# IDEA-CCNL/Fengshenbang-LM

Hardware: AMD Instinct MI355X
Metric: tokens/sec Ziya-LLaMA-13B ZeRO-3 (higher is better)
Workload: dtype bf16; 1 GPU; model=Ziya-LLaMA-13B, global_batch=16, micro_batch=16, seq_len=2048, parallelism=zero3_dp1, activation_checkpointing=True, ckpt_skip_interval=4

## Files before the change

### fengshen_amd/ops/csrc/bindings.cpp

```cpp
#include <torch/extension.h>

#include <hip/hip_runtime.h>
#include <c10/hip/HIPStream.h>

#include <string>
#include <vector>

enum FsDtype { FS_F32 = 0, FS_BF16 = 1, FS_F16 = 2 };

static int fs_dtype(const at::Tensor& t) {
  switch (t.scalar_type()) {
    case at::kFloat: return FS_F32;
    case at::kBFloat16: return FS_BF16;
    case at::kHalf: return FS_F16;
    default: TORCH_CHECK(false, "unsupported dtype ", t.scalar_type());
  }
}

static hipStream_t cur_stream() {
  return c10::hip::getCurrentHIPStream().stream();
}

extern "C" {
void fs_rms_norm_fwd(const void*, const void*, void*, float*, int, int, float,
                     int, hipStream_t);
void fs_rms_norm_bwd(const void*, const void*, const void*, const float*,
                     void*, float*, int, int, int, hipStream_t);
void fs_layer_norm_fwd(const void*, const void*, const void*, void*, float*,
                       float*, int, int, float, int, hipStream_t);
void fs_layer_norm_bwd(const void*, const void*, const void*, const float*,
                       const float*, void*, float*, float*, int, int, int,
                       hipStream_t);
void fs_scaled_softmax_fwd(const void*, const unsigned char*, void*, float,
                           int, int, int, int, int, int, int, int,
                           hipStream_t);
void fs_scaled_softmax_bwd(const void*, const void*, void*, float, int, int,
                           int, hipStream_t);
void fs_rope(const void*, void*, const float*, const float*, long, int, int,
             int, int, int, hipStream_t);
void fs_swiglu_fwd(const void*, void*, long, int, int, hipStream_t);
void fs_swiglu_bwd(const void*, const void*, void*, long, int, int,
                   hipStream_t);
void fs_bias_gelu(const void*, const void*, const void*, void*, long, int, int,
                  int, hipStream_t);
void fs_fused_adamw(float*, const void*, float*, float*, void*, long, float,
                    float, float, float, float, int, int, int, hipStream_t);
void fs_flash_attn_fwd(const void*, const void*, const void*, void*, float*,
                       const int*, int, int, int, int, int, int, float,
                       float, unsigned long long, hipStream_t);
void fs_flash_attn_bwd(const void*, const void*, const void*, const void*,
                       const void*, const float*, void*, void*, void*, float*,
                       const int*, int, int, int, int, int, int, float,
                       float, unsigned long long, hipStream_t);
void fs_bf16_gemv(const void*, const void*, void*, int, int, int,
                  hipStream_t);
void fs_add_rms_norm(const void*, const void*, const void*, void*, void*,
                     int, int, float, hipStream_t);
void fs_decode_attn(const void*, void*, void*, const float*, const float*,
                    const void*, void*, int, int, int, int, int, float, int,
                    hipStream_t);
void fs_w8_gemv(const void*, const float*, const void*, void*, int, int, int,
                hipStream_t);
void fs_vocab_ce_fwd(const void*, const long*, float*, float*, float*,
                     long, int, int, int, hipStream_t);
void fs_vocab_ce_bwd(const void*, const long*, const float*, const float*,
                     const float*, void*, long, int, int, int, hipStream_t);
void fs_flash_attn_fwd_v3(const void*, const void*, const void*, void*,
                          float*, const int*, int, int, int, int, int, float,
                          float, unsigned long long, hipStream_t);
void fs_flash_attn_bwd_v3(const void*, const void*, const void*, const void*,
                          const void*, const float*, void*, void*, void*,
                          float*, const int*, int, int, int, int, int, float,
                          float, unsigned long long, hipStream_t);
void fs_flash_attn_fwd_v3_strided(const void*, const void*, const void*,
                                  void*, float*, const int*, const long*,
                                  const long*, int, int, int, int, int, float,
                                  float, unsigned long long, hipStream_t);
void fs_flash_attn_bwd_v3_strided(const void*, const void*, const void*,
                                  const void*, const void*, const float*,
                                  void*, void*, void*, float*, const int*,
                                  const long*, const long*, const long*,
                                  const long*, int, int, int, int, int, float,
                                  float, unsigned long long, hipStream_t);
void fs_flash_attn_fwd_v3_kstart(const void*, const void*, const void*, void*,
                                 float*, const int*, const long*, const long*,
                                 int, int, int, int, float, hipStream_t);
void fs_flash_attn_bwd_v3_kstart(const void*, const void*, const void*,
                                 const void*, const void*, const float*,
                                 void*, void*, void*, float*, const int*,
// ... 497 lines not shown
  }
  if (kstart.has_value()) {
    fs_flash_attn_fwd_v3_kstart(q.data_ptr(), k.data_ptr(), v.data_ptr(),
                                o.data_ptr(), lse.data_ptr<float>(),
                                kstart->data_ptr<int>(), qs, os, b, h, s, d,
                                (float)scale, cur_stream());
    return lse;
  }
  fs_flash_attn_fwd_v3_strided(q.data_ptr(), k.data_ptr(), v.data_ptr(),
                               o.data_ptr(), lse.data_ptr<float>(), klp, qs,
                               os, b, h, s, d, causal ? 1 : 0, (float)scale,
                               0.f, 0ull, cur_stream());
  return lse;
}

static void flash_attn_bwd_v3_strided(
    at::Tensor q, at::Tensor k, at::Tensor v, at::Tensor o, at::Tensor dout,
    at::Tensor lse, at::Tensor dq, at::Tensor dk, at::Tensor dv, double scale,
    bool causal, c10::optional<at::Tensor> klens,
    c10::optional<at::Tensor> kstart, c10::optional<at::Tensor> qend,
    bool check_values) {
  TORCH_CHECK(q.dim() == 4, "q must be [b, h, s, d]");
  const int b = q.size(0), h = q.size(1), s = q.size(2), d = q.size(3);
  TORCH_CHECK((d == 128 || d == 96 || d == 64) && s % 64 == 0 && s >= 64,
              "flash v3: d in {64, 96, 128}, s a multiple of 64");
  const int h_kv = checked_kv_heads(k, h, causal, 0.0, klens.has_value());
  check_strided_view(q, "q", b, h, s, d);
  check_strided_view(k, "k", b, h_kv, s, d);
  check_strided_view(v, "v", b, h_kv, s, d);
  check_strided_view(o, "o", b, h, s, d);
  check_strided_view(dout, "dout", b, h, s, d);
  check_strided_view(dq, "dq", b, h, s, d);
  check_strided_view(dk, "dk", b, h_kv, s, d);
  check_strided_view(dv, "dv", b, h_kv, s, d);
  if (h_kv == h) {
    check_same_strides(q, k, "q and k");
    check_same_strides(dq, dk, "dq and dk");
  }
  check_same_strides(k, v, "k and v");
  check_same_strides(dk, dv, "dk and dv");
  TORCH_CHECK(lse.is_cuda() && lse.scalar_type() == at::kFloat &&
              lse.is_contiguous() && lse.numel() == (int64_t)b * h * s,
              "lse must be contiguous fp32 [b, h, s]");
  if (kstart.has_value())
    check_kstart(*kstart, qend, true, q, causal, 0.0, klens.has_value(),
                 check_values);
  else
    TORCH_CHECK(!qend.has_value(), "flash v3: qend without kstart");
  const int* klp = checked_klens(klens, causal, b);
  long qs[3], os[3], dos[3], gs[3];
  strides3(q, qs);
  strides3(o, os);
  strides3(dout, dos);
  strides3(dq, gs);
  auto delta = at::empty({b, h, s}, q.options().dtype(at::kFloat));
  if (h_kv != h) {
    long kvs[3], gkvs[3];
    strides3(k, kvs);
    strides3(dk, gkvs);
    const bool ks = kstart.has_value();
    fs_flash_attn_bwd_v3_gqa(
        q.data_ptr(), k.data_ptr(), v.data_ptr(), o.data_ptr(),
        dout.data_ptr(), lse.data_ptr<float>(), dq.data_ptr(), dk.data_ptr(),
        dv.data_ptr(), delta.data_ptr<float>(),
        ks ? kstart->data_ptr<int>() : nullptr,
        ks ? qend->data_ptr<int>() : nullptr, qs, kvs, os, dos, gs, gkvs, b,
        h, h_kv, s, d, (float)scale, cur_stream());
    return;
  }
  if (kstart.has_value()) {
    fs_flash_attn_bwd_v3_kstart(
        q.data_ptr(), k.data_ptr(), v.data_ptr(), o.data_ptr(),
        dout.data_ptr(), lse.data_ptr<float>(), dq.data_ptr(), dk.data_ptr(),
        dv.data_ptr(), delta.data_ptr<float>(), kstart->data_ptr<int>(),
        qend->data_ptr<int>(), qs, os, dos, gs, b, h, s, d, (float)scale,
        cur_stream());
    return;
  }
  fs_flash_attn_bwd_v3_strided(
      q.data_ptr(), k.data_ptr(), v.data_ptr(), o.data_ptr(), dout.data_ptr(),
      lse.data_ptr<float>(), dq.data_ptr(), dk.data_ptr(), dv.data_ptr(),
      delta.data_ptr<float>(), klp, qs, os, dos, gs, b, h, s, d,
      causal ? 1 : 0, (float)scale, 0.f, 0ull, cur_stream());
}

static void rope_inplace(at::Tensor q, at::Tensor k, at::Tensor cos,
                         at::Tensor sin, int64_t offset, bool bwd) {
  TORCH_CHECK(q.dim() == 4, "q must be [b, np, s, hn]");
  const int b = q.size(0), np = q.size(1), s = q.size(2), hn = q.size(3);
  TORCH_CHECK((hn / 2) % 8 == 0 && hn % 2 == 0,
              "head_dim/2 must be divisible by 8");
  check_strided_view(q, "q", b, np, s, hn);
  check_strided_view(k, "k", b, np, s, hn);
  check_same_strides(q, k, "q and k");
  TORCH_CHECK(cos.is_cuda() && sin.is_cuda() &&
              cos.scalar_type() == at::kFloat &&
              sin.scalar_type() == at::kFloat && cos.is_contiguous() &&
              sin.is_contiguous() && cos.dim() == 2 && cos.size(1) == hn &&
              sin.sizes() == cos.sizes(),
              "cos/sin must be contiguous fp32 [S, hn]");
  TORCH_CHECK(offset >= 0 && offset + s <= cos.size(0),
              "rope table too short for offset + s");
  fs_rope_inplace(q.data_ptr(), k.data_ptr(), cos.data_ptr<float>(),
                  sin.data_ptr<float>(), b, np, s, hn, q.stride(0),
                  q.stride(1), q.stride(2), (int)offset, bwd ? 1 : 0,
                  fs_dtype(q), cur_stream());
}

static void rope_inplace_one(at::Tensor x, at::Tensor cos, at::Tensor sin,
                             int64_t offset, bool bwd) {
  TORCH_CHECK(x.dim() == 4, "x must be [b, n, s, hn]");
  const int b = x.size(0), np = x.size(1), s = x.size(2), hn = x.size(3);
  TORCH_CHECK((hn / 2) % 8 == 0 && hn % 2 == 0,
              "head_dim/2 must be divisible by 8");
  check_strided_view(x, "x", b, np, s, hn);
  TORCH_CHECK(cos.is_cuda() && sin.is_cuda() &&
              cos.scalar_type() == at::kFloat &&
              sin.scalar_type() == at::kFloat && cos.is_contiguous() &&
              sin.is_contiguous() && cos.dim() == 2 && cos.size(1) == hn &&
              sin.sizes() == cos.sizes(),
              "cos/sin must be contiguous fp32 [S, hn]");
  TORCH_CHECK(offset >= 0 && offset + s <= cos.size(0),
              "rope table too short for offset + s");
  fs_rope_inplace(x.data_ptr(), nullptr, cos.data_ptr<float>(),
                  sin.data_ptr<float>(), b, np, s, hn, x.stride(0),
                  x.stride(1), x.stride(2), (int)offset, bwd ? 1 : 0,
                  fs_dtype(x), cur_stream());
}

static at::Tensor w8_gemv(at::Tensor q8, at::Tensor scale, at::Tensor x) {
  TORCH_CHECK(q8.scalar_type() == at::kChar && x.scalar_type() == at::kBFloat16);
  TORCH_CHECK(q8.is_contiguous() && x.is_contiguous());
  const int out = q8.size(0), in = q8.size(1);
  TORCH_CHECK(in % 16 == 0, "in_features must be divisible by 16");
  const int b = x.numel() / in;
  auto y = at::empty({b, out}, x.options());
  fs_w8_gemv(q8.data_ptr(), scale.data_ptr<float>(), x.data_ptr(),
             y.data_ptr(), b, in, out, cur_stream());
  return y;
}

static at::Tensor bf16_gemv(at::Tensor w, at::Tensor x) {
  TORCH_CHECK(w.scalar_type() == at::kBFloat16 &&
              x.scalar_type() == at::kBFloat16);
  TORCH_CHECK(w.is_contiguous() && x.is_contiguous());
  const int out = w.size(0), in = w.size(1);
  TORCH_CHECK(in % 16 == 0, "in_features must be divisible by 16");
  const int b = x.numel() / in;
  TORCH_CHECK(b >= 1 && b <= 8, "bf16_gemv: batch must be 1..8");
  auto y = at::empty({b, out}, x.options());
  fs_bf16_gemv(w.data_ptr(), x.data_ptr(), y.data_ptr(), b, in, out,
               cur_stream());
  return y;
}

static at::Tensor decode_attn(at::Tensor qkv, at::Tensor kc, at::Tensor vc,
                              at::Tensor cos_t, at::Tensor sin_t,
                              at::Tensor pos, double scale, bool rope) {
  TORCH_CHECK(qkv.scalar_type() == at::kBFloat16 && qkv.is_contiguous());
  TORCH_CHECK(kc.is_contiguous() && vc.is_contiguous());
  TORCH_CHECK(cos_t.scalar_type() == at::kFloat &&
              sin_t.scalar_type() == at::kFloat);
  TORCH_CHECK(pos.scalar_type() == at::kLong);
  TORCH_CHECK(kc.dim() == 4 && vc.sizes() == kc.sizes() &&
                  kc.scalar_type() == at::kBFloat16 &&
                  vc.scalar_type() == at::kBFloat16,
// ... 207 lines not shown
                                  c10::optional<at::Tensor> kstart,
                                  c10::optional<at::Tensor> qend,
                                  bool check_values) {
    const int b = q.size(0), h = q.size(1), s = q.size(2), d = q.size(3);
    TORCH_CHECK((d == 128 || d == 96 || d == 64) && s % 64 == 0);
    const bool gqa =
        checked_kv_heads(k, h, causal, drop_p, klens.has_value()) != h;
    if (kstart.has_value() || gqa) {
      TORCH_CHECK(drop_p == 0.0, "flash v3: kstart does not support dropout");
      TORCH_CHECK(q.is_contiguous() && k.is_contiguous() && v.is_contiguous());
      auto dq = at::empty_like(q);
      auto dk = at::empty_like(k);
      auto dv = at::empty_like(v);
      flash_attn_bwd_v3_strided(q, k, v, o, dout.contiguous(), lse, dq, dk,
                                dv, scale, causal, klens, kstart, qend,
                                check_values);
      return std::vector<at::Tensor>{dq, dk, dv};
    }
    TORCH_CHECK(!qend.has_value(), "flash v3: qend without kstart");
    const int* klp = nullptr;
    if (klens.has_value()) klp = klens->data_ptr<int>();
    auto dq = at::empty_like(q);
    auto dk = at::empty_like(k);
    auto dv = at::empty_like(v);
    auto delta = at::empty({b, h, s}, q.options().dtype(at::kFloat));
    fs_flash_attn_bwd_v3(q.data_ptr(), k.data_ptr(), v.data_ptr(),
                         o.data_ptr(), dout.contiguous().data_ptr(),
                         lse.data_ptr<float>(), dq.data_ptr(), dk.data_ptr(),
                         dv.data_ptr(), delta.data_ptr<float>(), klp, b, h,
                         s, d, causal ? 1 : 0, (float)scale, (float)drop_p,
                         (unsigned long long)seed, cur_stream());
    return std::vector<at::Tensor>{dq, dk, dv};
  }, py::arg("q"), py::arg("k"), py::arg("v"), py::arg("o"), py::arg("dout"),
     py::arg("lse"), py::arg("scale"), py::arg("causal"), py::arg("klens"),
     py::arg("drop_p"), py::arg("seed"), py::arg("kstart") = py::none(),
     py::arg("qend") = py::none(), py::arg("check_values") = false);
  mod.def("flash_attn_fwd_v3", [](at::Tensor q, at::Tensor k, at::Tensor v,
                                  double scale, bool causal,
                                  c10::optional<at::Tensor> klens,
                                  double drop_p, int64_t seed,
                                  c10::optional<at::Tensor> kstart,
                                  bool check_values) {
    TORCH_CHECK(q.is_contiguous() && k.is_contiguous() && v.is_contiguous());
    TORCH_CHECK(q.scalar_type() == at::kBFloat16);
    const int b = q.size(0), h = q.size(1), s = q.size(2), d = q.size(3);
    TORCH_CHECK((d == 128 || d == 96 || d == 64) && s % 64 == 0 && s >= 64);
    TORCH_CHECK(k.size(2) == s, "v3 is self-attention (sq == sk)");
    const bool gqa =
        checked_kv_heads(k, h, causal, drop_p, klens.has_value()) != h;
    if (kstart.has_value() || gqa) {
      TORCH_CHECK(drop_p == 0.0, "flash v3: kstart does not support dropout");
      auto o = at::empty_like(q);
      auto lse = flash_attn_fwd_v3_strided(q, k, v, o, scale, causal, klens,
                                           kstart, check_values);
      return std::vector<at::Tensor>{o, lse};
    }
    const int* klp = nullptr;
    if (klens.has_value()) {
      TORCH_CHECK(klens->scalar_type() == at::kInt
                  && klens->numel() == b && klens->is_contiguous());
      klp = klens->data_ptr<int>();
    }
    auto o = at::empty_like(q);
    auto lse = at::empty({b, h, s}, q.options().dtype(at::kFloat));
    fs_flash_attn_fwd_v3(q.data_ptr(), k.data_ptr(), v.data_ptr(),
                         o.data_ptr(), lse.data_ptr<float>(), klp, b, h, s,
                         d, causal ? 1 : 0, (float)scale, (float)drop_p,
                         (unsigned long long)seed, cur_stream());
    return std::vector<at::Tensor>{o, lse};
  }, py::arg("q"), py::arg("k"), py::arg("v"), py::arg("scale"),
     py::arg("causal"), py::arg("klens"), py::arg("drop_p"), py::arg("seed"),
     py::arg("kstart") = py::none(), py::arg("check_values") = false);
  mod.def("flash_attn_bwd", &flash_attn_bwd);
  mod.def("flash_attn_fwd_v3_strided", &flash_attn_fwd_v3_strided,
          py::arg("q"), py::arg("k"), py::arg("v"), py::arg("o"),
          py::arg("scale"), py::arg("causal"), py::arg("klens"),
          py::arg("kstart") = py::none(), py::arg("check_values") = false);
  mod.def("flash_attn_bwd_v3_strided", &flash_attn_bwd_v3_strided,
          py::arg("q"), py::arg("k"), py::arg("v"), py::arg("o"),
          py::arg("dout"), py::arg("lse"), py::arg("dq"), py::arg("dk"),
          py::arg("dv"), py::arg("scale"), py::arg("causal"),
          py::arg("klens"), py::arg("kstart") = py::none(),
          py::arg("qend") = py::none(), py::arg("check_values") = false);
  mod.def("rope_inplace", &rope_inplace);
  mod.def("rope_inplace_one", &rope_inplace_one);
  mod.def("rms_norm_fwd", &rms_norm_fwd);
  mod.def("rms_norm_bwd", &rms_norm_bwd);
  mod.def("residual_rms_norm_fwd", &residual_rms_norm_fwd);
  mod.def("residual_rms_norm_bwd", &residual_rms_norm_bwd);
  mod.def("fused_norm_branch", &fused_norm_branch);
  mod.def("layer_norm_fwd", &layer_norm_fwd);
  mod.def("layer_norm_bwd", &layer_norm_bwd);
  mod.def("scaled_masked_softmax_fwd", &scaled_masked_softmax_fwd);
  mod.def("scaled_causal_softmax_fwd", &scaled_causal_softmax_fwd);
  mod.def("scaled_softmax_bwd", &scaled_softmax_bwd);
  mod.def("rope_fwd", &rope_fwd);
  mod.def("rope_bwd", &rope_bwd);
  mod.def("swiglu_fwd", &swiglu_fwd);
  mod.def("swiglu_bwd", &swiglu_bwd);
  mod.def("bias_gelu_fwd", &bias_gelu_fwd);
  mod.def("bias_gelu_bwd", &bias_gelu_bwd);
  mod.def("fused_adamw", &fused_adamw);
}
```

### fengshen_amd/ops/csrc/flash_attn.hip

```cpp

#include "common.h"

typedef __attribute__((ext_vector_type(8))) short bf16x8;
typedef __attribute__((ext_vector_type(4))) float f32x4;

#define FA_QBLK 128
#define FA_KVBLK 64
#define FA_WAVES 8
#define FA_VPAD 8
#define FB_T 32

constexpr int fa_dpad(int d) { return (d + 31) / 32 * 32; }
constexpr int fa_swb(int dp) {
  int need = 2 * dp, p = 128;
  while (p < need) p <<= 1;
  return p;
}

__device__ __forceinline__ int kswz(int row, int byte_in_row) {
  return byte_in_row ^ ((row & 7) << 4);
}

__device__ __forceinline__ unsigned int fa_hash(unsigned long long seed,
                                                unsigned long long idx) {
  unsigned long long z = seed + idx * 0x9E3779B97F4A7C15ull;
  z = (z ^ (z >> 30)) * 0xBF58476D1CE4E5B9ull;
  z = (z ^ (z >> 27)) * 0x94D049BB133111EBull;
  return (unsigned int)(z >> 32);
}

__device__ __forceinline__ short fa_bf16bits(float f) {
  return (short)__hip_bfloat16_raw(__float2bfloat16(f)).x;
}

template <int D>
__device__ __forceinline__ bf16x8 fa_load8(const bf16_t* rowp, int d0) {
  if (d0 < D) return *reinterpret_cast<const bf16x8*>(rowp + d0);
  bf16x8 z;
#pragma unroll
  for (int j = 0; j < 8; ++j) z[j] = 0;
  return z;
}

template <int D, bool CAUSAL>
__global__ __launch_bounds__(FA_WAVES * 64)
void flash_attn_fwd_kernel(const bf16_t* __restrict__ Q,
                           const bf16_t* __restrict__ K,
                           const bf16_t* __restrict__ V,
                           bf16_t* __restrict__ O,
                           float* __restrict__ LSE,
                           const int* __restrict__ klens,
                           int b, int h, int sq, int sk, float scale,
                           unsigned int drop_thresh, float keep_scale,
                           unsigned long long drop_seed) {
  constexpr int DP = fa_dpad(D);
  constexpr int NC = DP / 32;
  constexpr int NTO = DP / 16;
  constexpr int SWB = fa_swb(DP);

  __shared__ char k_raw[FA_KVBLK * SWB];
  __shared__ short vt_lds[DP][FA_KVBLK + FA_VPAD];
  __shared__ short p_lds[FA_WAVES][16][FA_KVBLK + FA_VPAD];

  const int lane = threadIdx.x & 63;
  const int wave = threadIdx.x >> 6;
  const int qb = blockIdx.x;
  const int head = blockIdx.y;
  const int batch = blockIdx.z;

  const bf16_t* Qp = Q + ((long)batch * h + head) * sq * D;
  const bf16_t* Kp = K + ((long)batch * h + head) * sk * D;
  const bf16_t* Vp = V + ((long)batch * h + head) * sk * D;
  bf16_t* Op = O + ((long)batch * h + head) * sq * D;

  const int klen = CAUSAL ? sk
                          : min(klens ? klens[batch] : sk, sk);

  const int q0 = qb * FA_QBLK + wave * 16;
  const bool q_active = q0 < sq;
  const int q0c = q_active ? q0 : (sq > 16 ? sq - 16 : 0);

  bf16x8 q_frag[NC];
  {
    const int row = lane & 15;
// ... 798 lines not shown
                                  unsigned long long seed,
                                  hipStream_t stream) {
  const unsigned int dth =
      (drop_p > 0.f) ? (unsigned int)(drop_p * 4294967296.0) : 0u;
  const float ksc = (drop_p > 0.f) ? 1.f / (1.f - drop_p) : 1.f;
#define BWD_CASE(DD) case DD: launch_bwd<DD>(causal, q, k, v, o, dout, lse, \
    dq, dk, dv, delta_ws, klens, b, h, sq, sk, scale, dth, ksc, seed, \
    stream); break;
  switch (d) {
    BWD_CASE(40) BWD_CASE(64) BWD_CASE(80)
    BWD_CASE(96) BWD_CASE(128) BWD_CASE(160)
  }
#undef BWD_CASE
}


#define V3_QBLK 256
#define V3_KVBLK 64

typedef __attribute__((ext_vector_type(16))) float f32x16;

struct FaStrides {
  long b, h, r;
};

typedef __attribute__((ext_vector_type(4))) short bf16x4;
typedef __attribute__((address_space(3))) bf16x4 lds_bf16x4;

template <int SWB>
__device__ __forceinline__ int v3_off(int row, int ch) {
  static_assert(SWB == 256 || SWB == 128, "row stride");
  if (SWB == 256)
    return 256 * row + 16 * (ch ^ (((row & 3) << 2) | ((row >> 2) & 3)));
  return 128 * row + 16 * (ch ^ ((((row >> 1) & 1) << 2) | ((row >> 2) & 3)));
}

template <int SWB>
__device__ __forceinline__ int v3_tr_addr(int lane, int row0, int col0) {
  const int i = lane & 15;
  const int col = col0 + 16 * ((lane >> 4) & 1) + 4 * (i & 3);
  return v3_off<SWB>(row0 + (i >> 2), col >> 3) + 2 * (col & 7);
}

__device__ __forceinline__ bf16x8 v3_tr_frag(const char* a0, const char* a1) {
  const bf16x4 lo = __builtin_amdgcn_ds_read_tr16_b64_v4i16((lds_bf16x4*)a0);
  const bf16x4 hi = __builtin_amdgcn_ds_read_tr16_b64_v4i16((lds_bf16x4*)a1);
  return __builtin_shufflevector(lo, hi, 0, 1, 2, 3, 4, 5, 6, 7);
}

template <int SWB>
__device__ __forceinline__ bf16x8 v3_tr_bfrag(const char* rows, int tbase,
                                              int t) {
  const int a0 = tbase ^ (64 * t);
  return v3_tr_frag(rows + a0, rows + (a0 ^ 16) + 4 * SWB);
}

__device__ __forceinline__ void v3_wait_lds() {
  __builtin_amdgcn_s_waitcnt(0xC07F);
}

__device__ __forceinline__ int dkv_xoff(int row, int u) {
  return 64 * row + 8 * (u ^ ((row >> 1) & 7));
}

__device__ __forceinline__ int v3_kstart_at(const int* ksb, int row) {
  return min(max(ksb[row], 0), row);
}

__device__ __forceinline__ int v3_wave_min(int v) {
#pragma unroll
  for (int o = 32; o > 0; o >>= 1) v = min(v, __shfl_xor(v, o, 64));
  return __builtin_amdgcn_readfirstlane(v);
}

__device__ __forceinline__ int v3_block_kstart_min(const int* ksb, int blk,
                                                   int lane, int s) {
  int m = s;
#pragma unroll
  for (int j = 0; j < V3_QBLK / 64; ++j)
    m = min(m, v3_kstart_at(ksb, min(blk * V3_QBLK + 64 * j + lane, s - 1)));
  return v3_wave_min(m);
}


template <int D>
__global__ __launch_bounds__(256)
void flash_delta_v3_kernel(const bf16_t* __restrict__ dO,
                           const bf16_t* __restrict__ O,
                           float* __restrict__ delta, FaStrides dos,
                           FaStrides os, int h, int s) {
  const int lane = threadIdx.x & 63;
  const int wid = threadIdx.x >> 6;
  const bf16_t* dob = dO + blockIdx.z * dos.b + blockIdx.y * dos.h;
  const bf16_t* ob = O + blockIdx.z * os.b + blockIdx.y * os.h;
  float* dl = delta + ((long)blockIdx.z * h + blockIdx.y) * s;
  for (int row = blockIdx.x * 4 + wid; row < s; row += gridDim.x * 4) {
    const bf16_t* dop = dob + row * dos.r;
    const bf16_t* op = ob + row * os.r;
    float sacc = 0.f;
    for (int i = lane * 2; i < D; i += 128) {
#pragma unroll
      for (int j = 0; j < 2; ++j)
        sacc += __bfloat162float(dop[i + j]) * __bfloat162float(op[i + j]);
    }
    sacc = wave_reduce_sum(sacc);
    if (lane == 0) dl[row] = sacc;
  }
}

template <int D, bool CAUSAL, bool HAS_DROP, bool KS = false,
          bool GQA = false>
__global__ __launch_bounds__(FA_WAVES * 64)
void flash_attn_fwd_v3_kernel(const bf16_t* __restrict__ Q,
                              const bf16_t* __restrict__ K,
                              const bf16_t* __restrict__ V,
                              bf16_t* __restrict__ O,
                              float* __restrict__ LSE,
                              const int* __restrict__ klens,
                              FaStrides qs, FaStrides os,
                              int b, int h, int s, float scale,
                              unsigned int drop_thresh, float keep_scale,
                              unsigned long long drop_seed,
                              const int* __restrict__ kstart,
                              FaStrides kvs, int G) {
  static_assert(!KS || (CAUSAL && !HAS_DROP), "kstart: causal, no dropout");
  static_assert(!GQA || (CAUSAL && !HAS_DROP), "GQA: causal, no dropout");
  constexpr int NC = D / 16;
  constexpr int NTO = D / 32;
  constexpr int SWB = fa_swb(D);

  __shared__ __attribute__((aligned(16)))
  char k_raw[2][V3_KVBLK * SWB];
  __shared__ __attribute__((aligned(16)))
  char v_raw[2][V3_KVBLK * SWB];

  const int lane = threadIdx.x & 63;
  const int wave = threadIdx.x >> 6;
  const int hi = lane >> 5;
  const int ln = lane & 31;
  const long bh = (long)blockIdx.z * h + blockIdx.y;
  const long qoff = blockIdx.z * qs.b + blockIdx.y * qs.h;
  const bf16_t* Qp = Q + qoff;
  const long kvoff =
      GQA ? blockIdx.z * kvs.b + (blockIdx.y / G) * kvs.h : qoff;
  const long kv_r = GQA ? kvs.r : qs.r;
  const bf16_t* Kp = K + kvoff;
  const bf16_t* Vp = V + kvoff;
  bf16_t* Op = O + blockIdx.z * os.b + blockIdx.y * os.h;

  const int klen = CAUSAL ? s : min(klens ? klens[blockIdx.z] : s, s);

  const int q0w = blockIdx.x * V3_QBLK + wave * 32;
  const bool q_active = q0w < s;
  const int q0c = q_active ? q0w : s - 32;
  const int my_q = q0c + ln;

  bf16x8 q_frag[NC];
#pragma unroll
  for (int c = 0; c < NC; ++c) {
    bf16x8 raw = *reinterpret_cast<const bf16x8*>(
        Qp + (long)my_q * qs.r + c * 16 + hi * 8);
#pragma unroll
    for (int j = 0; j < 8; ++j) {
      unsigned short u = (unsigned short)raw[j];
      float f = __uint_as_float(((unsigned int)u) << 16) * scale;
      raw[j] = fa_bf16bits(f);
    }
    q_frag[c] = raw;
  }

  int ks_q = 0, ks_w = 0, kt0 = 0;
  if (KS) {
    const int* ksb = kstart + (long)blockIdx.z * s;
    ks_q = v3_kstart_at(ksb, my_q);
    ks_w = v3_wave_min(ks_q);
    kt0 = v3_block_kstart_min(ksb, blockIdx.x, lane, s) / V3_KVBLK;
  }

  float m_run = KS ? -1e30f : -INFINITY, l_run = 0.f;
  f32x16 o_acc[NTO];
#pragma unroll
  for (int t = 0; t < NTO; ++t) {
#pragma unroll
    for (int r = 0; r < 16; ++r) o_acc[t][r] = 0.f;
  }

  int n_kv_tiles;
  if (CAUSAL) {
    const int q_hi_row = min(blockIdx.x * V3_QBLK + V3_QBLK, s) - 1;
    n_kv_tiles = (q_hi_row / V3_KVBLK) + 1;
  } else {
    n_kv_tiles = (klen + V3_KVBLK - 1) / V3_KVBLK;
    if (n_kv_tiles < 1) n_kv_tiles = 1;
  }

  const int tid = threadIdx.x;
  constexpr int ELEMS = V3_KVBLK * D;
  constexpr int SWEEPS = (ELEMS + FA_WAVES * 64 * 8 - 1) / (FA_WAVES * 64 * 8);
  bf16x8 k_reg[SWEEPS], v_reg[SWEEPS];
#pragma unroll
  for (int sweep = 0; sweep < SWEEPS; ++sweep) {
    const int i = tid * 8 + sweep * (FA_WAVES * 64 * 8);
    if (i < ELEMS) {
      const long kr = KS ? min(kt0 * V3_KVBLK + i / D, s - 1)
                         : min(i / D, s - 1);
      const int kc = i % D;
      k_reg[sweep] = *reinterpret_cast<const bf16x8*>(Kp + kr * kv_r + kc);
      v_reg[sweep] = *reinterpret_cast<const bf16x8*>(Vp + kr * kv_r + kc);
    }
  }

  {
#pragma unroll
    for (int sweep = 0; sweep < SWEEPS; ++sweep) {
      const int i = tid * 8 + sweep * (FA_WAVES * 64 * 8);
      if (i < ELEMS) {
        const int kr = i / D;
        const int kc = i % D;
        *reinterpret_cast<bf16x8*>(
            k_raw[0] + kr * SWB + kswz(kr, kc * 2)) = k_reg[sweep];
        *reinterpret_cast<bf16x8*>(
            v_raw[0] + v3_off<SWB>(kr, kc >> 3)) = v_reg[sweep];
      }
    }
  }
  const int v_tr = v3_tr_addr<SWB>(lane, 8 * hi, 0);
  const int q_last_w = __builtin_amdgcn_readfirstlane(q0c) + 31;

  int cur = 0;
  for (int kt = KS ? kt0 : 0; kt < n_kv_tiles; ++kt) {
    const int k_base = kt * V3_KVBLK;
    __syncthreads();
    if (kt + 1 < n_kv_tiles) {
      const int nb = (kt + 1) * V3_KVBLK;
#pragma unroll
      for (int sweep = 0; sweep < SWEEPS; ++sweep) {
        const int i = tid * 8 + sweep * (FA_WAVES * 64 * 8);
        if (i < ELEMS) {
          const long kr = min((long)(nb + i / D), (long)s - 1);
          const int kc = i % D;
          k_reg[sweep] = *reinterpret_cast<const bf16x8*>(Kp + kr * kv_r + kc);
          v_reg[sweep] = *reinterpret_cast<const bf16x8*>(Vp + kr * kv_r + kc);
        }
      }
    }

    if ((!CAUSAL || k_base <= q_last_w) &&
        (!KS || k_base + V3_KVBLK > ks_w)) {
      f32x16 st[2];
#pragma unroll
      for (int nt = 0; nt < 2; ++nt) {
#pragma unroll
        for (int r = 0; r < 16; ++r) st[nt][r] = 0.f;
      }
#pragma unroll
      for (int nt = 0; nt < 2; ++nt) {
        const int krow = nt * 32 + ln;
#pragma unroll
        for (int c = 0; c < NC; ++c) {
          bf16x8 a = *reinterpret_cast<const bf16x8*>(
              k_raw[cur] + krow * SWB + kswz(krow, (c * 16 + hi * 8) * 2));
          st[nt] = __builtin_amdgcn_mfma_f32_32x32x16_bf16(a, q_frag[c],
                                                           st[nt], 0, 0, 0);
        }
      }

      float p[32];
      float tmax = -INFINITY;
#pragma unroll
      for (int nt = 0; nt < 2; ++nt) {
#pragma unroll
        for (int r = 0; r < 16; ++r) {
// ... 166 lines not shown
  dim3 block(FA_WAVES * 64);
#define V3K(DD) hipLaunchKernelGGL( \
    (flash_attn_fwd_v3_kernel<DD, true, false, true>), \
    grid, block, 0, stream, (const bf16_t*)q, (const bf16_t*)k, \
    (const bf16_t*)v, (bf16_t*)o, lse, (const int*)nullptr, qs, os, b, h, s, \
    scale, 0u, 1.f, 0ull, kstart, FaStrides{}, 1)
  if (d == 128) V3K(128);
  else if (d == 96) V3K(96);
  else V3K(64);
#undef V3K
}

extern "C" void fs_flash_attn_fwd_v3_gqa(
    const void* q, const void* k, const void* v, void* o, float* lse,
    const int* kstart, const long* qs3, const long* kvs3, const long* os3,
    int b, int h, int h_kv, int s, int d, float scale, hipStream_t stream) {
  const FaStrides qs{qs3[0], qs3[1], qs3[2]};
  const FaStrides kvs{kvs3[0], kvs3[1], kvs3[2]};
  const FaStrides os{os3[0], os3[1], os3[2]};
  dim3 grid((s + V3_QBLK - 1) / V3_QBLK, h, b);
  dim3 block(FA_WAVES * 64);
#define V3G(DD, KK) hipLaunchKernelGGL( \
    (flash_attn_fwd_v3_kernel<DD, true, false, KK, true>), \
    grid, block, 0, stream, (const bf16_t*)q, (const bf16_t*)k, \
    (const bf16_t*)v, (bf16_t*)o, lse, (const int*)nullptr, qs, os, b, h, s, \
    scale, 0u, 1.f, 0ull, kstart, kvs, h / h_kv)
  if (kstart) {
    if (d == 128) V3G(128, true);
    else if (d == 96) V3G(96, true);
    else V3G(64, true);
  } else {
    if (d == 128) V3G(128, false);
    else if (d == 96) V3G(96, false);
    else V3G(64, false);
  }
#undef V3G
}

extern "C" void fs_flash_attn_fwd_v3(const void* q, const void* k,
                                     const void* v, void* o, float* lse,
                                     const int* klens, int b, int h, int s,
                                     int d, int causal, float scale,
                                     float drop_p, unsigned long long seed,
                                     hipStream_t stream) {
  const long c3[3] = {(long)h * s * d, (long)s * d, (long)d};
  fs_flash_attn_fwd_v3_strided(q, k, v, o, lse, klens, c3, c3, b, h, s, d,
                               causal, scale, drop_p, seed, stream);
}


#define B3_FB 32

template <int D, bool CAUSAL, bool HAS_DROP, bool KS = false,
          bool GQA = false>
__global__ __launch_bounds__(FA_WAVES * 64)
void flash_attn_bwd_dq_v3_kernel(const bf16_t* __restrict__ Q,
                                 const bf16_t* __restrict__ K,
                                 const bf16_t* __restrict__ V,
                                 const bf16_t* __restrict__ dO,
                                 const float* __restrict__ LSE,
                                 const float* __restrict__ Delta,
                                 bf16_t* __restrict__ dQ,
                                 const int* __restrict__ klens,
                                 FaStrides qs, FaStrides dos, FaStrides gs,
                                 int b, int h, int s, float scale,
                                 unsigned int drop_thresh, float keep_scale,
                                 unsigned long long drop_seed,
                                 const int* __restrict__ kstart,
                                 FaStrides kvs, int G) {
  static_assert(!KS || (CAUSAL && !HAS_DROP), "kstart: causal, no dropout");
  static_assert(!GQA || (CAUSAL && !HAS_DROP), "GQA: causal, no dropout");
  constexpr int NC = D / 16;
  constexpr int NTO = D / 32;
  constexpr int SWB = fa_swb(D);

  __shared__ __attribute__((aligned(16))) char k_raw[2][B3_FB * SWB];
  __shared__ __attribute__((aligned(16))) char v_raw[2][B3_FB * SWB];
  __shared__ short p_x[FA_WAVES][32][B3_FB + FA_VPAD];

  const int lane = threadIdx.x & 63;
  const int wave = threadIdx.x >> 6;
  const int hi = lane >> 5;
  const int ln = lane & 31;
  const long bh = (long)blockIdx.z * h + blockIdx.y;
  const long qoff = blockIdx.z * qs.b + blockIdx.y * qs.h;
  const bf16_t* Qp = Q + qoff;
  const long kvoff =
      GQA ? blockIdx.z * kvs.b + (blockIdx.y / G) * kvs.h : qoff;
  const long kv_r = GQA ? kvs.r : qs.r;
  const bf16_t* Kp = K + kvoff;
  const bf16_t* Vp = V + kvoff;
  const bf16_t* dOp = dO + blockIdx.z * dos.b + blockIdx.y * dos.h;
  bf16_t* dQp = dQ + blockIdx.z * gs.b + blockIdx.y * gs.h;
  const float* lse = LSE + bh * s;
  const float* dlt = Delta + bh * s;

  const int klen = CAUSAL ? s : min(klens ? klens[blockIdx.z] : s, s);
  const int q0w = blockIdx.x * V3_QBLK + wave * 32;
  const bool q_active = q0w < s;
  const int q0c = q_active ? q0w : s - 32;
  const int my_q = q0c + ln;

  bf16x8 q_frag[NC], do_frag[NC];
#pragma unroll
  for (int c = 0; c < NC; ++c) {
    bf16x8 raw = *reinterpret_cast<const bf16x8*>(
        Qp + (long)my_q * qs.r + c * 16 + hi * 8);
#pragma unroll
    for (int j = 0; j < 8; ++j) {
      unsigned short u = (unsigned short)raw[j];
      raw[j] = fa_bf16bits(
          __uint_as_float(((unsigned int)u) << 16) * scale);
    }
    q_frag[c] = raw;
    do_frag[c] = *reinterpret_cast<const bf16x8*>(
        dOp + (long)my_q * dos.r + c * 16 + hi * 8);
  }
  const float lse_r = lse[my_q];
  const float dlt_r = dlt[my_q];
  int ks_q = 0, ks_w = 0, kt0 = 0;
  if (KS) {
    const int* ksb = kstart + (long)blockIdx.z * s;
    ks_q = v3_kstart_at(ksb, my_q);
    ks_w = v3_wave_min(ks_q);
    kt0 = v3_block_kstart_min(ksb, blockIdx.x, lane, s) / B3_FB;
  }

  f32x16 dq_acc[NTO];
#pragma unroll
  for (int t = 0; t < NTO; ++t) {
#pragma unroll
    for (int r = 0; r < 16; ++r) dq_acc[t][r] = 0.f;
  }

  int n_kv_tiles;
  if (CAUSAL) {
    const int q_hi_row = min(blockIdx.x * V3_QBLK + V3_QBLK, s) - 1;
    n_kv_tiles = (q_hi_row / B3_FB) + 1;
  } else {
    n_kv_tiles = (klen + B3_FB - 1) / B3_FB;
  }

  const int st_i = threadIdx.x * 8;
  const bool st_on = st_i < B3_FB * D;
  const int st_r = st_on ? st_i / D : 0;
  const int st_c = st_on ? st_i % D : 0;
  const int st_off = v3_off<SWB>(st_r, st_c >> 3);
  bf16x8 k_reg, v_reg;
  {
    const long krg = KS ? min(kt0 * B3_FB + st_r, s - 1) : min(st_r, s - 1);
    k_reg = *reinterpret_cast<const bf16x8*>(Kp + krg * kv_r + st_c);
    v_reg = *reinterpret_cast<const bf16x8*>(Vp + krg * kv_r + st_c);
  }
  if (st_on) {
    *reinterpret_cast<bf16x8*>(k_raw[0] + st_off) = k_reg;
    *reinterpret_cast<bf16x8*>(v_raw[0] + st_off) = v_reg;
  }
  const int k_tr = v3_tr_addr<SWB>(lane, 8 * hi, 0);
  const int kv_row = v3_off<SWB>(ln, hi);
  const int q_last_w = __builtin_amdgcn_readfirstlane(q0c) + 31;

  int cur = 0;
  for (int kt = KS ? kt0 : 0; kt < n_kv_tiles; ++kt) {
    const int k_base = kt * B3_FB;
    __syncthreads();
    if (kt + 1 < n_kv_tiles) {
      const long krg = min(k_base + B3_FB + st_r, s - 1);
      k_reg = *reinterpret_cast<const bf16x8*>(Kp + krg * kv_r + st_c);
      v_reg = *reinterpret_cast<const bf16x8*>(Vp + krg * kv_r + st_c);
    }

    if ((!CAUSAL || k_base <= q_last_w) && (!KS || k_base + B3_FB > ks_w)) {
      f32x16 st, dpt;
#pragma unroll
      for (int r = 0; r < 16; ++r) {
        st[r] = 0.f;
        dpt[r] = 0.f;
      }
      {
#pragma unroll
        for (int c = 0; c < NC; ++c) {
          const int roff = kv_row ^ (32 * c);
          bf16x8 ka = *reinterpret_cast<const bf16x8*>(k_raw[cur] + roff);
          st = __builtin_amdgcn_mfma_f32_32x32x16_bf16(ka, q_frag[c], st,
                                                       0, 0, 0);
          bf16x8 va = *reinterpret_cast<const bf16x8*>(v_raw[cur] + roff);
          dpt = __builtin_amdgcn_mfma_f32_32x32x16_bf16(va, do_frag[c], dpt,
                                                        0, 0, 0);
        }
      }

#pragma unroll
      for (int g = 0; g < 4; ++g) {
        short pk[4] __attribute__((aligned(8)));
#pragma unroll
        for (int j = 0; j < 4; ++j) {
          const int r = g * 4 + j;
          const int kcol = k_base + (r & 3) + 8 * (r >> 2) + 4 * hi;
          const bool masked = CAUSAL ? (kcol > my_q || (KS && kcol < ks_q))
                                     : (kcol >= klen);
          float pv = masked ? 0.f : __expf(st[r] - lse_r);
          float dpv = dpt[r];
          if (HAS_DROP && drop_thresh) {
            const unsigned long long idx =
                (bh * (unsigned long long)s + my_q) *
                    (unsigned long long)s + kcol;
            dpv = (fa_hash(drop_seed, idx) < drop_thresh)
                      ? 0.f : dpv * keep_scale;
          }
          pk[j] = fa_bf16bits(pv * (dpv - dlt_r) * scale);
        }
        *reinterpret_cast<long*>(&p_x[wave][ln][8 * g + 4 * hi]) =
            *reinterpret_cast<const long*>(pk);
      }
      v3_wait_lds();

#pragma unroll
      for (int c2 = 0; c2 < 2; ++c2) {
        bf16x8 pa = *reinterpret_cast<const bf16x8*>(
            &p_x[wave][ln][c2 * 16 + hi * 8]);
        const char* krows = k_raw[cur] + c2 * 16 * SWB;
#pragma unroll
        for (int t = 0; t < NTO; ++t) {
          bf16x8 kb = v3_tr_bfrag<SWB>(krows, k_tr, t);
          dq_acc[t] = __builtin_amdgcn_mfma_f32_32x32x16_bf16(pa, kb,
                                                              dq_acc[t],
                                                              0, 0, 0);
        }
      }
    }

    if (kt + 1 < n_kv_tiles) {
      cur ^= 1;
      if (st_on) {
        *reinterpret_cast<bf16x8*>(k_raw[cur] + st_off) = k_reg;
        *reinterpret_cast<bf16x8*>(v_raw[cur] + st_off) = v_reg;
      }
    }
  }

  if (!q_active) return;
#pragma unroll
  for (int r = 0; r < 16; ++r) {
    const int qrow = q0w + (r & 3) + 8 * (r >> 2) + 4 * hi;
#pragma unroll
    for (int t = 0; t < NTO; ++t)
      dQp[(long)qrow * gs.r + t * 32 + ln] = __float2bfloat16(dq_acc[t][r]);
  }
}

template <int D, bool CAUSAL, bool HAS_DROP, bool KS = false,
          bool GQA = false>
__global__ __launch_bounds__(FA_WAVES * 64)
void flash_attn_bwd_dkv_v3_kernel(const bf16_t* __restrict__ Q,
                                  const bf16_t* __restrict__ K,
                                  const bf16_t* __restrict__ V,
                                  const bf16_t* __restrict__ dO,
                                  const float* __restrict__ LSE,
                                  const float* __restrict__ Delta,
                                  bf16_t* __restrict__ dK,
                                  bf16_t* __restrict__ dV,
                                  const int* __restrict__ klens,
                                  FaStrides qs, FaStrides dos, FaStrides gs,
                                  int b, int h, int s, float scale,
                                  unsigned int drop_thresh, float keep_scale,
                                  unsigned long long drop_seed,
                                  const int* __restrict__ kstart,
                                  const int* __restrict__ qend,
                                  FaStrides kvs, FaStrides gkvs, int G) {
  static_assert(!KS || (CAUSAL && !HAS_DROP), "kstart: causal, no dropout");
  static_assert(!GQA || (CAUSAL && !HAS_DROP), "GQA: causal, no dropout");
  constexpr int NC = D / 16;
  constexpr int NTO = D / 32;
  constexpr int SWB = fa_swb(D);

  __shared__ __attribute__((aligned(16))) char q_raw[B3_FB * SWB];
  __shared__ __attribute__((aligned(16))) char do_raw[B3_FB * SWB];
  __shared__ __attribute__((aligned(16))) char p_x[FA_WAVES][32 * 64];
  __shared__ __attribute__((aligned(16))) char ds_x[FA_WAVES][32 * 64];

  const int lane = threadIdx.x & 63;
  const int wave = threadIdx.x >> 6;
  const int hi = lane >> 5;
  const int ln = lane & 31;
  const unsigned int qh0 = GQA ? blockIdx.y * G : blockIdx.y;
  const long bh = (long)blockIdx.z * h + qh0;
  const long qoff = blockIdx.z * qs.b + qh0 * qs.h;
  const bf16_t* Qp = Q + qoff;
  const long kvoff = GQA ? blockIdx.z * kvs.b + blockIdx.y * kvs.h : qoff;
  const long kv_r = GQA ? kvs.r : qs.r;
  const bf16_t* Kp = K + kvoff;
  const bf16_t* Vp = V + kvoff;
  const bf16_t* dOp = dO + blockIdx.z * dos.b + qh0 * dos.h;
  const long goff = GQA ? blockIdx.z * gkvs.b + blockIdx.y * gkvs.h
                        : blockIdx.z * gs.b + blockIdx.y * gs.h;
  const long g_r = GQA ? gkvs.r : gs.r;
  bf16_t* dKp = dK + goff;
  bf16_t* dVp = dV + goff;
  const float* lse = LSE + bh * s;
  const float* dlt = Delta + bh * s;

  const int klen = CAUSAL ? s : min(klens ? klens[blockIdx.z] : s, s);
  const int kv0_blk = blockIdx.x * V3_QBLK;
  const int kv0w = kv0_blk + wave * 32;
  const bool kv_active = kv0w < s;
  const int kv0c = kv_active ? kv0w : s - 32;
  const int my_kv = kv0c + ln;

  f32x16 dv_acc[NTO], dk_acc[NTO];
#pragma unroll
  for (int t = 0; t < NTO; ++t) {
#pragma unroll
    for (int r = 0; r < 16; ++r) {
      dv_acc[t][r] = 0.f;
      dk_acc[t][r] = 0.f;
    }
  }

  const int first_qt = CAUSAL ? kv0_blk / B3_FB : 0;
  int n_q_tiles = s / B3_FB;
  const int* ksb = nullptr;
  if (KS) {
    ksb = kstart + (long)blockIdx.z * s;
    const int nt = s / V3_KVBLK;
    const int* qe = qend + (long)blockIdx.z * nt;
    int e = 0;
#pragma unroll
    for (int j = 0; j < V3_QBLK / V3_KVBLK; ++j)
      e = max(e, qe[min(kv0_blk / V3_KVBLK + j, nt - 1)]);
    n_q_tiles = min(max(e, kv0_blk), s - 1) / B3_FB + 1;
  }

  const int st_i = threadIdx.x * 8;
  const bool st_on = st_i < B3_FB * D;
  const int st_r = st_on ? st_i / D : 0;
  const int st_c = st_on ? st_i % D : 0;
  const int st_off = v3_off<SWB>(st_r, st_c >> 3);
  const int qd_tr = v3_tr_addr<SWB>(lane, 8 * hi, 0);
  const int qd_row = v3_off<SWB>(ln, hi);
  int x_tr[2];
#pragma unroll
  for (int e = 0; e < 2; ++e) {
    const int i = lane & 15;
    const int row = 8 * hi + 4 * e + (i >> 2);
    x_tr[e] = dkv_xoff(row, 4 * ((lane >> 4) & 1) + (i & 3));
  }
  bf16x8 k_frag[NC], v_frag[NC];
#pragma unroll
  for (int c = 0; c < NC; ++c) {
    k_frag[c] = *reinterpret_cast<const bf16x8*>(
        Kp + (long)my_kv * kv_r + c * 16 + hi * 8);
    v_frag[c] = *reinterpret_cast<const bf16x8*>(
        Vp + (long)my_kv * kv_r + c * 16 + hi * 8);
  }

  int gm = 0;
  for (int qt = first_qt; qt < n_q_tiles; ++qt) {
    const int q_base = qt * B3_FB;
    __syncthreads();
    {
      const long qrg = q_base + st_r;
      const bf16x8 qq =
          *reinterpret_cast<const bf16x8*>(Qp + qrg * qs.r + st_c);
      const bf16x8 dd =
          *reinterpret_cast<const bf16x8*>(dOp + qrg * dos.r + st_c);
      if (st_on) {
        *reinterpret_cast<bf16x8*>(q_raw + st_off) = qq;
        *reinterpret_cast<bf16x8*>(do_raw + st_off) = dd;
      }
    }
    const int qcol = q_base + ln;
    const float lse_c = lse[qcol];
    const float dlt_c = dlt[qcol];
    int ks_c = 0;
    if (KS) ks_c = v3_kstart_at(ksb, qcol);
    __syncthreads();

    f32x16 st, dpt;
#pragma unroll
    for (int r = 0; r < 16; ++r) st[r] = 0.f;
#pragma unroll
    for (int c = 0; c < NC; ++c) {
      bf16x8 qb = *reinterpret_cast<const bf16x8*>(
          q_raw + (qd_row ^ (32 * c)));
      st = __builtin_amdgcn_mfma_f32_32x32x16_bf16(k_frag[c], qb, st, 0, 0,
                                                   0);
    }
#pragma unroll
    for (int r = 0; r < 16; ++r) dpt[r] = 0.f;
#pragma unroll
    for (int c = 0; c < NC; ++c) {
      bf16x8 db = *reinterpret_cast<const bf16x8*>(
          do_raw + (qd_row ^ (32 * c)));
      dpt = __builtin_amdgcn_mfma_f32_32x32x16_bf16(v_frag[c], db, dpt, 0, 0,
                                                    0);
    }

#pragma unroll
    for (int g = 0; g < 4; ++g) {
      short pk[4] __attribute__((aligned(8)));
      short dk4[4] __attribute__((aligned(8)));
#pragma unroll
      for (int j = 0; j < 4; ++j) {
        const int r = g * 4 + j;
        const int kvrow = kv0c + (r & 3) + 8 * (r >> 2) + 4 * hi;
        const bool masked = CAUSAL ? (qcol < kvrow || (KS && kvrow < ks_c))
                                   : (kvrow >= klen);
        float pv = masked ? 0.f : __expf(st[r] * scale - lse_c);
// ... 223 lines not shown
```

Baseline: 10450 tokens/s.

## Remap flash attention v3 block indices for XCD-local L2 reuse and heavy-first order

Adds a block-index remapping so that consecutive linear block ids, which are dispatched round-robin across the 8 XCDs, are assigned contiguous (head, q-tile) ranges per XCD. Blocks sharing K/V for the same head then land on the same XCD's L2. The forward and dQ kernels also reverse the x order so the heaviest causal tiles are scheduled first, improving load balance. A host binding exposes the map for testing. The cost is a few integer divides per block, and the scheme assumes 8 XCDs.

```diff
diff --git a/fengshen_amd/ops/csrc/bindings.cpp b/fengshen_amd/ops/csrc/bindings.cpp
--- a/fengshen_amd/ops/csrc/bindings.cpp
+++ b/fengshen_amd/ops/csrc/bindings.cpp
@@ -5,6 +5,8 @@
 
 #include <string>
 #include <vector>
+
+#include "flash_blockmap.h"
 
 enum FsDtype { FS_F32 = 0, FS_BF16 = 1, FS_F16 = 2 };
 
@@ -668,6 +670,24 @@
       lse.data_ptr<float>(), dq.data_ptr(), dk.data_ptr(), dv.data_ptr(),
       delta.data_ptr<float>(), klp, qs, os, dos, gs, b, h, s, d,
       causal ? 1 : 0, (float)scale, 0.f, 0ull, cur_stream());
+}
+
+static at::Tensor flash_v3_block_map(int64_t nx, int64_t ny, int64_t nz,
+                                     bool heavy_last) {
+  TORCH_CHECK(nx >= 1 && ny >= 1 && nz >= 1 && nx * ny * nz <= (1 << 24),
+              "flash_v3_block_map: grid (", nx, ", ", ny, ", ", nz, ")");
+  const int64_t T = nx * ny * nz;
+  auto out = at::empty({T, 3}, at::TensorOptions().dtype(at::kInt));
+  int* p = out.data_ptr<int>();
+  for (int64_t L = 0; L < T; ++L) {
+    const FlashBlock blk = flash_v3_block_of(
+        (unsigned int)L, (unsigned int)nx, (unsigned int)ny, (unsigned int)nz,
+        heavy_last);
+    p[3 * L + 0] = (int)blk.x;
+    p[3 * L + 1] = (int)blk.y;
+    p[3 * L + 2] = (int)blk.z;
+  }
+  return out;
 }
 
 static void rope_inplace(at::Tensor q, at::Tensor k, at::Tensor cos,
@@ -1041,6 +1061,8 @@
           py::arg("dv"), py::arg("scale"), py::arg("causal"),
           py::arg("klens"), py::arg("kstart") = py::none(),
           py::arg("qend") = py::none(), py::arg("check_values") = false);
+  mod.def("flash_v3_block_map", &flash_v3_block_map, py::arg("nx"),
+          py::arg("ny"), py::arg("nz"), py::arg("heavy_last"));
   mod.def("rope_inplace", &rope_inplace);
   mod.def("rope_inplace_one", &rope_inplace_one);
   mod.def("rms_norm_fwd", &rms_norm_fwd);
diff --git a/fengshen_amd/ops/csrc/flash_attn.hip b/fengshen_amd/ops/csrc/flash_attn.hip
--- a/fengshen_amd/ops/csrc/flash_attn.hip
+++ b/fengshen_amd/ops/csrc/flash_attn.hip
@@ -1,5 +1,6 @@
 
 #include "common.h"
+#include "flash_blockmap.h"
 
 typedef __attribute__((ext_vector_type(8))) short bf16x8;
 typedef __attribute__((ext_vector_type(4))) float f32x4;
@@ -964,6 +965,12 @@
   return v3_wave_min(m);
 }
 
+__device__ __forceinline__ FlashBlock v3_block(bool heavy_last) {
+  const unsigned int L =
+      blockIdx.x + gridDim.x * (blockIdx.y + gridDim.y * blockIdx.z);
+  return flash_v3_block_of(L, gridDim.x, gridDim.y, gridDim.z, heavy_last);
+}
+
 
 template <int D>
 __global__ __launch_bounds__(256)
@@ -1020,19 +1027,21 @@
   const int wave = threadIdx.x >> 6;
   const int hi = lane >> 5;
   const int ln = lane & 31;
-  const long bh = (long)blockIdx.z * h + blockIdx.y;
-  const long qoff = blockIdx.z * qs.b + blockIdx.y * qs.h;
+  const FlashBlock blk = v3_block(true);
+  const unsigned int bx = blk.x, by = blk.y, bz = blk.z;
+  const long bh = (long)bz * h + by;
+  const long qoff = bz * qs.b + by * qs.h;
   const bf16_t* Qp = Q + qoff;
   const long kvoff =
-      GQA ? blockIdx.z * kvs.b + (blockIdx.y / G) * kvs.h : qoff;
+      GQA ? bz * kvs.b + (by / G) * kvs.h : qoff;
   const long kv_r = GQA ? kvs.r : qs.r;
   const bf16_t* Kp = K + kvoff;
   const bf16_t* Vp = V + kvoff;
-  bf16_t* Op = O + blockIdx.z * os.b + blockIdx.y * os.h;
-
-  const int klen = CAUSAL ? s : min(klens ? klens[blockIdx.z] : s, s);
-
-  const int q0w = blockIdx.x * V3_QBLK + wave * 32;
+  bf16_t* Op = O + bz * os.b + by * os.h;
+
+  const int klen = CAUSAL ? s : min(klens ? klens[bz] : s, s);
+
+  const int q0w = bx * V3_QBLK + wave * 32;
   const bool q_active = q0w < s;
   const int q0c = q_active ? q0w : s - 32;
   const int my_q = q0c + ln;
@@ -1053,10 +1062,10 @@
 
   int ks_q = 0, ks_w = 0, kt0 = 0;
   if (KS) {
-    const int* ksb = kstart + (long)blockIdx.z * s;
+    const int* ksb = kstart + (long)bz * s;
     ks_q = v3_kstart_at(ksb, my_q);
     ks_w = v3_wave_min(ks_q);
-    kt0 = v3_block_kstart_min(ksb, blockIdx.x, lane, s) / V3_KVBLK;
+    kt0 = v3_block_kstart_min(ksb, bx, lane, s) / V3_KVBLK;
   }
 
   float m_run = KS ? -1e30f : -INFINITY, l_run = 0.f;
@@ -1069,7 +1078,7 @@
 
   int n_kv_tiles;
   if (CAUSAL) {
-    const int q_hi_row = min(blockIdx.x * V3_QBLK + V3_QBLK, s) - 1;
+    const int q_hi_row = min(bx * V3_QBLK + V3_QBLK, s) - 1;
     n_kv_tiles = (q_hi_row / V3_KVBLK) + 1;
   } else {
     n_kv_tiles = (klen + V3_KVBLK - 1) / V3_KVBLK;
@@ -1402,21 +1411,23 @@
   const int wave = threadIdx.x >> 6;
   const int hi = lane >> 5;
   const int ln = lane & 31;
-  const long bh = (long)blockIdx.z * h + blockIdx.y;
-  const long qoff = blockIdx.z * qs.b + blockIdx.y * qs.h;
+  const FlashBlock blk = v3_block(true);
+  const unsigned int bx = blk.x, by = blk.y, bz = blk.z;
+  const long bh = (long)bz * h + by;
+  const long qoff = bz * qs.b + by * qs.h;
   const bf16_t* Qp = Q + qoff;
   const long kvoff =
-      GQA ? blockIdx.z * kvs.b + (blockIdx.y / G) * kvs.h : qoff;
+      GQA ? bz * kvs.b + (by / G) * kvs.h : qoff;
   const long kv_r = GQA ? kvs.r : qs.r;
   const bf16_t* Kp = K + kvoff;
   const bf16_t* Vp = V + kvoff;
-  const bf16_t* dOp = dO + blockIdx.z * dos.b + blockIdx.y * dos.h;
-  bf16_t* dQp = dQ + blockIdx.z * gs.b + blockIdx.y * gs.h;
+  const bf16_t* dOp = dO + bz * dos.b + by * dos.h;
+  bf16_t* dQp = dQ + bz * gs.b + by * gs.h;
   const float* lse = LSE + bh * s;
   const float* dlt = Delta + bh * s;
 
-  const int klen = CAUSAL ? s : min(klens ? klens[blockIdx.z] : s, s);
-  const int q0w = blockIdx.x * V3_QBLK + wave * 32;
+  const int klen = CAUSAL ? s : min(klens ? klens[bz] : s, s);
+  const int q0w = bx * V3_QBLK + wave * 32;
   const bool q_active = q0w < s;
   const int q0c = q_active ? q0w : s - 32;
   const int my_q = q0c + ln;
@@ -1440,10 +1451,10 @@
   const float dlt_r = dlt[my_q];
   int ks_q = 0, ks_w = 0, kt0 = 0;
   if (KS) {
-    const int* ksb = kstart + (long)blockIdx.z * s;
+    const int* ksb = kstart + (long)bz * s;
     ks_q = v3_kstart_at(ksb, my_q);
     ks_w = v3_wave_min(ks_q);
-    kt0 = v3_block_kstart_min(ksb, blockIdx.x, lane, s) / B3_FB;
+    kt0 = v3_block_kstart_min(ksb, bx, lane, s) / B3_FB;
   }
 
   f32x16 dq_acc[NTO];
@@ -1455,7 +1466,7 @@
 
   int n_kv_tiles;
   if (CAUSAL) {
-    const int q_hi_row = min(blockIdx.x * V3_QBLK + V3_QBLK, s) - 1;
+    const int q_hi_row = min(bx * V3_QBLK + V3_QBLK, s) - 1;
     n_kv_tiles = (q_hi_row / B3_FB) + 1;
   } else {
     n_kv_tiles = (klen + B3_FB - 1) / B3_FB;
@@ -1603,25 +1614,27 @@
   const int wave = threadIdx.x >> 6;
   const int hi = lane >> 5;
   const int ln = lane & 31;
-  const unsigned int qh0 = GQA ? blockIdx.y * G : blockIdx.y;
-  const long bh = (long)blockIdx.z * h + qh0;
-  const long qoff = blockIdx.z * qs.b + qh0 * qs.h;
+  const FlashBlock blk = v3_block(false);
+  const unsigned int bx = blk.x, by = blk.y, bz = blk.z;
+  const unsigned int qh0 = GQA ? by * G : by;
+  const long bh = (long)bz * h + qh0;
+  const long qoff = bz * qs.b + qh0 * qs.h;
   const bf16_t* Qp = Q + qoff;
-  const long kvoff = GQA ? blockIdx.z * kvs.b + blockIdx.y * kvs.h : qoff;
+  const long kvoff = GQA ? bz * kvs.b + by * kvs.h : qoff;
   const long kv_r = GQA ? kvs.r : qs.r;
   const bf16_t* Kp = K + kvoff;
   const bf16_t* Vp = V + kvoff;
-  const bf16_t* dOp = dO + blockIdx.z * dos.b + qh0 * dos.h;
-  const long goff = GQA ? blockIdx.z * gkvs.b + blockIdx.y * gkvs.h
-                        : blockIdx.z * gs.b + blockIdx.y * gs.h;
+  const bf16_t* dOp = dO + bz * dos.b + qh0 * dos.h;
+  const long goff = GQA ? bz * gkvs.b + by * gkvs.h
+                        : bz * gs.b + by * gs.h;
   const long g_r = GQA ? gkvs.r : gs.r;
   bf16_t* dKp = dK + goff;
   bf16_t* dVp = dV + goff;
   const float* lse = LSE + bh * s;
   const float* dlt = Delta + bh * s;
 
-  const int klen = CAUSAL ? s : min(klens ? klens[blockIdx.z] : s, s);
-  const int kv0_blk = blockIdx.x * V3_QBLK;
+  const int klen = CAUSAL ? s : min(klens ? klens[bz] : s, s);
+  const int kv0_blk = bx * V3_QBLK;
   const int kv0w = kv0_blk + wave * 32;
   const bool kv_active = kv0w < s;
   const int kv0c = kv_active ? kv0w : s - 32;
@@ -1641,9 +1654,9 @@
   int n_q_tiles = s / B3_FB;
   const int* ksb = nullptr;
   if (KS) {
-    ksb = kstart + (long)blockIdx.z * s;
+    ksb = kstart + (long)bz * s;
     const int nt = s / V3_KVBLK;
-    const int* qe = qend + (long)blockIdx.z * nt;
+    const int* qe = qend + (long)bz * nt;
     int e = 0;
 #pragma unroll
     for (int j = 0; j < V3_QBLK / V3_KVBLK; ++j)
diff --git a/fengshen_amd/ops/csrc/flash_blockmap.h b/fengshen_amd/ops/csrc/flash_blockmap.h
--- /dev/null
+++ b/fengshen_amd/ops/csrc/flash_blockmap.h
@@ -0,0 +1,30 @@
+#pragma once
+
+#if defined(__HIPCC__)
+#define FLASH_HD __host__ __device__
+#else
+#define FLASH_HD
+#endif
+
+#define FLASH_NXCD 8
+
+struct FlashBlock {
+  unsigned int x, y, z;
+};
+
+FLASH_HD inline FlashBlock flash_v3_block_of(unsigned int L, unsigned int nx,
+                                             unsigned int ny, unsigned int nz,
+                                             bool heavy_last) {
+  const unsigned int T = nx * ny * nz;
+  const unsigned int q = T / FLASH_NXCD, r = T % FLASH_NXCD;
+  const unsigned int label = L % FLASH_NXCD, slot = L / FLASH_NXCD;
+  const unsigned int first =
+      label < r ? label * (q + 1) : r * (q + 1) + (label - r) * q;
+  const unsigned int p = first + slot;
+  const unsigned int col = p / nx, i = p % nx;
+  FlashBlock blk;
+  blk.x = heavy_last ? nx - 1 - i : i;
+  blk.y = col % ny;
+  blk.z = col / ny;
+  return blk;
+}
```

Measured after the change: 10900 tokens/s, median of 6. 1.04x the previous value.
